# buwantaiji/FermiFlow

Hardware: AMD Instinct MI355X
Metric: walker-steps/sec (full VMC iteration: 100 MCMC steps + generate + E_loc + grad + Adam) (higher is better)
Workload: dtype f64

## Files before the change

### fermiflow_amd/csrc/ff_cnf_fwd.hip

```cpp
#include <atomic>
#include "ff_common.h"
#include "ff_ode.h"
#include "ff_slater.h"
#include "ff_eloc_ws.h"
#define FF_RADIAL_BUILD_KERNELS
#include "ff_radial.h"

#ifdef FF_STAMPS
#define FF_STAMP(i) do { unsigned long long t_ = __builtin_amdgcn_s_memtime(); stamp_acc[i] += t_ - stamp_prev; stamp_prev = t_; } while (0)
#else
#define FF_STAMP(i) do { } while (0)
#endif

#ifndef FF_TAB_MODE
#define FF_TAB_MODE(MODE) true
#endif

#include "ff_fwd_args.h"

#ifndef FF_FORM_EARLY
#define FF_FORM_EARLY 1
#endif
#ifndef FF_SWEEP_CH
#define FF_SWEEP_CH 2
#endif
#ifndef FF_FWD_WAVES_PER_SIMD
#define FF_FWD_WAVES_PER_SIMD 1
#endif
#ifndef FF_FLOW_WAVES
#define FF_FLOW_WAVES 3
#endif
#ifndef FF_FWD_STATIC
#define FF_FWD_STATIC(N, D, MODE, TAB) ((MODE) == 0 && (TAB) && (N) * (D) <= 12)
#endif
template <int N, int D, int MODE_, bool TAB>
__global__ void __launch_bounds__(FF_WAVE, ((MODE_ == 0 || MODE_ == FF_MODE_FRAMES) && TAB && N * D <= 12) ? FF_FLOW_WAVES : FF_FWD_WAVES_PER_SIMD)
ff_ode_fwd_kernel(ff_fwd_args A) {
  constexpr bool FRAMES = MODE_ == FF_MODE_FRAMES;
  constexpr int MODE = FRAMES ? 0 : MODE_;
  if constexpr (MODE == 0) FF_SETPRIO();
  using Gm = ff_geom<N, D>;
  constexpr int M = Gm::M, G = Gm::G, P = Gm::P, R = Gm::RA;
  constexpr int NH = MODE == 0 ? 1 : (MODE == 1 ? 2 : 4);
  constexpr int NV = MODE == 0 ? 1 : (MODE == 1 ? 2 : M + 5);
  constexpr int IDL = MODE == 1 ? 1 : M + 3;

  __shared__ ff_wtab s_w[TAB ? 1 : 2][TAB ? 1 : FF_HPAD];
  __shared__ double s_e2[TAB ? 1 : 64];
  __shared__ double s_z[G][M], s_kb[G][M], s_err[G][M];
  constexpr bool JET = (MODE == 2);
  __shared__ __attribute__((aligned(16))) double s_rr[JET ? 1 : G][JET ? 1 : R][2];
  __shared__ __attribute__((aligned(16))) double s_hd[JET ? 1 : G][JET ? 1 : R][NH];
  constexpr int RECW = (D + 7 + 1) & ~1;
  constexpr int RECS0 = R * RECW, RECS = RECS0 + ((RECS0 % 4 == 2) ? 0 : ((RECS0 % 4 == 0) ? 2 : 1));
  static_assert(!JET || ((2 * RECS) % 32) % 8 == 4, "record stride");
  __shared__ __attribute__((aligned(16))) double s_rec[JET ? G * RECS : 1];
  constexpr int QTW = ((3 * N > M) ? 3 * N + 1 : M + 1) | 1;
  constexpr int TROW = N * 3 * D + 1;
  static_assert(N * TROW <= M * QTW, "T must fit the transposition buffer");
  __shared__ __attribute__((aligned(16))) double s_qt[JET ? G * M * QTW : 1];
  __shared__ int s_pa[R], s_pb[R], s_any;
  __shared__ double s_rmin[G][R];
  static_assert(MODE != 2 || M <= 12, "the column-sweep local-energy kernel serves at most 12 coordinates");
  constexpr bool LDS_STATE = (MODE == 2);
  __shared__ double s_yv[LDS_STATE ? NV : 1][FF_WAVE], s_cv[LDS_STATE ? NV : 1][FF_WAVE];

  const int lane = threadIdx.x;
  const int g = lane / M, i = lane % M;
  const bool ingrp = g < G;
  const int gg = ingrp ? g : 0;
  const int ai = i / D, ci = i % D;
  const double* __restrict__ rtab = A.net.radial_table;
  if constexpr (TAB) {
    if (rtab[3] != 0.0) {
      if (lane == 0 && blockIdx.x == 0) *A.evt = A.evt_id;
      return;
    }
  } else {
    if (A.evt && *A.evt != A.evt_id) return;
    ff_fill_exp2_table(s_e2, lane);
    ff_load_weights(s_w, A.net, lane);
  }
  bool off_table = false;
  if (lane == 0) {
    int p = 0;
    for (int a = 0; a < N; a++)
      for (int b = a + 1; b < N; b++) { s_pa[p] = a; s_pb[p] = b; p++; }
    for (int a = 0; a < N; a++) { if (P + a < R) { s_pa[P + a] = a; s_pb[P + a] = -1; } }
  }
  FF_WG1_SYNC();
  const int He = A.net.He, Hm = A.net.Hm;
  const bool has_mu = Hm > 0;
  const int nrad = has_mu ? (P + N) : P;
  const double tab_inv_h = TAB ? rtab[0] : 0.0, tab_h = TAB ? rtab[1] : 0.0;
  auto heads = [&](int t, double r, double* hd) {
    if constexpr (TAB) {
      if (!ff_heads_table<NH>(rtab, tab_inv_h, tab_h, t, r, hd)) {
        off_table = true;
#pragma unroll
        for (int m = 0; m < NH; m++) hd[m] = 0.0;
      }
    } else {
      ff_heads<NH, FF_TAB_MODE(MODE)>(s_w[t], s_e2, t ? Hm : He, r, hd);
    }
  };
  const double rtol = A.rtol, atol = A.atol;
  constexpr double NT = MODE == 0 ? M : (MODE == 1 ? M + 1 : M * (M + 4) + 1);
  const int64_t ngroups = (A.B + G - 1) / G;
  __shared__ int s_st[4];
  if (lane < 4) s_st[lane] = 0;
  constexpr int NQ = (G * R + FF_WAVE - 1) / FF_WAVE;
  int rq_id[NQ];
#pragma unroll
  for (int qk = 0; qk < NQ; qk++) {
    const int q = lane + qk * FF_WAVE;
    const bool act = q < G * nrad;
// ... 74 lines not shown
        case 2: g0 = h * FF_A20; g1 = h * FF_A21; break;
        case 3: g0 = h * FF_A30; g1 = h * FF_A31; g2 = h * FF_A32; break;
        case 4: gy = 0.0; g0 = 1.0; break;
        case 5: gy = 0.0; g1 = 1.0; break;
        case 6: gy = 0.0; g2 = 1.0; break;
        default: break;
      }
      auto form = [&](double* dst, const int v0, const int v1, const int stride) {
#pragma unroll
        for (int v = v0; v < v1; v += stride) dst[v] = fma(g2, c2[v], fma(g1, c1[v], fma(g0, c0[v], gy * y[v])));
      };
      FF_STAMP(0);
      FF_WG1_SYNC();
      {
        double pub[NV];
        form(pub, 0, MODE == 2 ? M + 2 : 1, MODE == 2 ? M + 1 : 1);
        if (ingrp) {
          s_z[g][i] = pub[0];
          if constexpr (MODE == 2) s_kb[g][i] = pub[M + 1];
        }
      }
      FF_WG1_SYNC();
      FF_STAMP(1);
      double rq_rho[NQ][D], rq_dk[JET ? NQ : 1][D], rq_r[NQ], rq_ri[NQ], rq_T[NQ][TAB ? NH + 5 : 1], rq_dr[NQ];
      bool rq_ok[NQ];
#pragma unroll
      for (int qk = 0; qk < NQ; qk++) {
        const int id = rq_id[qk];
        const bool act = id >= 0;
        const int qg = act ? (id & 15) : 0, a = act ? ((id >> 4) & 15) : 0, bq = act ? ((id >> 8) & 15) : 15;
        const bool pair = bq != 15;
        const int bb = pair ? bq : a;
        double r2 = 0.0;
#pragma unroll
        for (int c = 0; c < D; c++) {
          rq_rho[qk][c] = s_z[qg][a * D + c] - (pair ? s_z[qg][bb * D + c] : 0.0);
          if constexpr (JET) rq_dk[qk][c] = s_kb[qg][a * D + c] - (pair ? s_kb[qg][bb * D + c] : 0.0);
          r2 = fma(rq_rho[qk][c], rq_rho[qk][c], r2);
        }
        ff_sqrt_rcp(r2, rq_r[qk], rq_ri[qk]);
        if (act) rmin_q[qk] = fmin(rmin_q[qk], rq_r[qk]);
        rq_dr[qk] = 0.0;
        rq_ok[qk] = true;
        if constexpr (TAB) {
          rq_ok[qk] = ff_table_fetch<NH>(rtab, tab_inv_h, tab_h, pair ? 0 : 1, rq_r[qk], rq_T[qk], rq_dr[qk]);
          if (act && !rq_ok[qk]) off_table = true;
        }
      }
      double in[NV], out[NV];
      if constexpr (MODE == 2 && FF_FORM_EARLY) form(in, 0, NV, 1);
#pragma unroll
      for (int qk = 0; qk < NQ; qk++) {
        const int id = rq_id[qk];
        if (id < 0) break;
        const int qg = id & 15, a = (id >> 4) & 15, bq = (id >> 8) & 15, p = id >> 12;
        const bool pair = bq != 15;
        const int bb = pair ? bq : a;
        const double* rho = rq_rho[qk];
        const double r = rq_r[qk], ri = rq_ri[qk];
        double hd[NH];
        if constexpr (TAB) {
          if (rq_ok[qk]) ff_table_eval<NH>(rq_T[qk], rq_dr[qk], hd);
          else {
#pragma unroll
            for (int m = 0; m < NH; m++) hd[m] = 0.0;
          }
        } else {
          heads(pair ? 0 : 1, r, hd);
        }
        if constexpr (!JET) {
          s_rr[qg][p][0] = r;
          s_rr[qg][p][1] = ri;
#pragma unroll
          for (int m = 0; m < NH; m++) s_hd[qg][p][m] = hd[m];
        } else {
          const double cf = pair ? 2.0 : 1.0;
          const double f0 = hd[0], f1 = hd[1], f2 = hd[NH > 2 ? 2 : 0], f3 = hd[NH > 3 ? 3 : 0];
          const double Ac = cf * fma(f2, r, (1.0 + D) * f1), Bc = cf * fma(f3, r, (2.0 + D) * f2);
          double* rec = &s_rec[qg * RECS + p * RECW];
#pragma unroll
          for (int c = 0; c < D; c++) rec[c] = rho[c];
          rec[D] = ri; rec[D + 1] = f0; rec[D + 2] = f1; rec[D + 3] = f2; rec[D + 4] = Ac; rec[D + 5] = Bc;
          rec[D + 6] = cf * fma(f1, r, D * f0);
          const double* dk = rq_dk[qk];
          double rdk = 0.0;
#pragma unroll
          for (int c = 0; c < D; c++) rdk = fma(rho[c], dk[c], rdk);
          const double F1k = f1 * (rdk * ri), gq = Ac * ri;
          double* Ta = &s_qt[qg * M * QTW + a * TROW + bb * 3 * D];
          double* Tb = &s_qt[qg * M * QTW + bb * TROW + a * 3 * D];
#pragma unroll
          for (int c = 0; c < D; c++) {
            const double pv = f0 * rho[c], pw = fma(F1k, rho[c], f0 * dk[c]), pg = gq * rho[c];
            Ta[c] = pv; Ta[D + c] = pw; Ta[2 * D + c] = pg;
            if (pair) { Tb[c] = -pv; Tb[D + c] = -pw; Tb[2 * D + c] = -pg; }
          }
        }
      }
      FF_WG1_SYNC();
      nev++;
      FF_STAMP(2);
      if constexpr (!(MODE == 2 && FF_FORM_EARLY)) form(in, 0, NV, 1);
      FF_STAMP(6);
      const double* sz = s_z[gg];
      double sumq = 0.0, ddiv = 0.0, qdiv = 0.0, divv = 0.0;
// ... 58 lines not shown
                if (pair) { du[bq * D + cc] -= g1; qv[bq * D + cc] -= g2; }
              }
              ddiv = fma(Ac, r1, ddiv);
              qdiv = fma(Bc, r1s, fma(Ac, r2q, qdiv));
              divv += hq[D + 6];
            }
          }
          FF_SCHED_FENCE();
        }
        FF_STAMP(7);
#pragma unroll
        for (int k = 0; k < M; k++) out[1 + k] = du[k];
        if (ingrp) {
#pragma unroll
          for (int k = 0; k < M; k++) s_qt[(g * M + i) * QTW + k] = qv[k];
        }
        FF_WG1_SYNC();
#pragma unroll
        for (int j = 0; j < M; j++) sumq += s_qt[(gg * M + j) * QTW + i];
        FF_STAMP(3);
      } else {
        if constexpr (MODE == 1) {
          for (int p = 0; p < nrad; p++) {
            const double c = p < P ? 2.0 : 1.0;
            divv = fma(c, fma(s_hd[gg][p][NH > 1 ? 1 : 0], s_rr[gg][p][0], D * s_hd[gg][p][0]), divv);
          }
        }
        const double zc = sz[ai * D + ci];
#pragma unroll
        for (int bq = 0; bq < N; bq++) {
          const bool self = (bq == ai);
          const int lo = bq < ai ? bq : ai, hi = bq < ai ? ai : bq;
          const int p = self ? 0 : ff_pair_index(N, lo, hi);
          vi = fma(self ? 0.0 : s_hd[gg][p][0], zc - sz[bq * D + ci], vi);
        }
        if (has_mu) vi = fma(s_hd[gg][P + ai][0], zc, vi);
      }
      out[0] = vi;
      if constexpr (MODE == 1) out[1] = -divv;
      if constexpr (MODE == 2) {
        out[M + 1] = sumq + dvk;
        out[M + 2] = -ddiv;
        out[M + 3] = -divv;
        out[M + 4] = -fma(gdi, in[M + 1], qdiv);
      }
      FF_STAMP(4);
#if defined(FF_STAMPS) && defined(FF_STAMPS_TRACE)
      const int s_prev = sv;
#endif
      if (sv == -2) {
#pragma unroll
        for (int v = 0; v < NV; v++) c0[v] = out[v];
        double p0 = 0.0, p1 = 0.0;
#pragma unroll
        for (int v = 0; v < NV; v++) {
          const double isc = wgt(v) * ff_rcp(fma(fabs(y[v]), rtol, atol));
          p0 = fma(y[v] * isc, y[v] * isc, p0);
          p1 = fma(c0[v] * isc, c0[v] * isc, p1);
        }
        const double d0 = sqrt(group_sum(p0) * (1.0 / NT));
        d1v = sqrt(group_sum(p1) * (1.0 / NT));
        h0v = S.h0(d0, d1v);
        s = -1;
        if (!ff_wave_or(&s_any, lane, (!S.done && !warm) ? 1 : 0)) {
          S.habs = fmin(hwarm, S.interval);
          S.plan();
          s = 1;
// ... 1165 lines not shown
```

### fermiflow_amd/csrc/ff_common.h

```cpp
#pragma once
#include <stdint.h>
#include <math.h>
#include "../../include/fermiflow.h"

#define FF_WAVE 64
#define FF_MAX_ORB 36
#define FF_MAX_NS 12
#define FF_HMAX 256
#define FF_HPAD (FF_HMAX + 8)

#ifdef FF_HOSTSIM
#include "../../tests/hostsim/hip_shim.h"
#else
#include <hip/hip_runtime.h>
#define FF_LAUNCH(kernel, grid, block, stream, ...) \
  hipLaunchKernelGGL(kernel, dim3(grid), dim3(block), 0, (hipStream_t)(stream), __VA_ARGS__)
#define FF_LAUNCH_LDS(kernel, grid, block, lds_bytes, stream, ...) \
  hipLaunchKernelGGL(kernel, dim3(grid), dim3(block), (lds_bytes), (hipStream_t)(stream), __VA_ARGS__)
#define FF_DYN_LDS(name) extern __shared__ double name[]
#endif

#ifndef FF_WAVE_SYNC
#define FF_WAVE_SYNC() do { __builtin_amdgcn_fence(__ATOMIC_RELEASE, "workgroup"); __builtin_amdgcn_wave_barrier(); \
                            __builtin_amdgcn_fence(__ATOMIC_ACQUIRE, "workgroup"); } while (0)
// ... 287 lines not shown
  p = fma(p, z, 1.0 / 3.0);
  p = fma(p, z, 1.0);
  const double ef = (double)e;
  return fma(ef, 6.93147180369123816490e-01, fma(2.0 * s, p, ef * 1.90821492927058770002e-10));
}

FF_D void ff_sincospi(double t, double* sn, double* cs) {
  const double q = rint(t * 2.0);
  const double r = fma(q, -0.5, t) * 3.14159265358979323846;
  const double r2 = r * r;
  double ps = -1.0 / 1307674368000.0;
  ps = fma(ps, r2, 1.0 / 6227020800.0);
  ps = fma(ps, r2, -1.0 / 39916800.0);
  ps = fma(ps, r2, 1.0 / 362880.0);
  ps = fma(ps, r2, -1.0 / 5040.0);
  ps = fma(ps, r2, 1.0 / 120.0);
  ps = fma(ps, r2, -1.0 / 6.0);
  ps = fma(ps * r2, r, r);
  double pc = 1.0 / 20922789888000.0;
  pc = fma(pc, r2, -1.0 / 87178291200.0);
  pc = fma(pc, r2, 1.0 / 479001600.0);
  pc = fma(pc, r2, -1.0 / 3628800.0);
  pc = fma(pc, r2, 1.0 / 40320.0);
  pc = fma(pc, r2, -1.0 / 720.0);
  pc = fma(pc, r2, 1.0 / 24.0);
  pc = fma(pc, r2, -0.5);
  pc = fma(pc, r2, 1.0);
  const int k = ((int)q) & 3;
  const double s0 = (k & 1) ? pc : ps, c0 = (k & 1) ? ps : pc;
  *sn = (k & 2) ? -s0 : s0;
  *cs = ((k + 1) & 2) ? -c0 : c0;
}

FF_HD int ff_pair_index(int n, int i, int j) { return i * (2 * n - i - 1) / 2 + (j - i - 1); }
```

### fermiflow_amd/csrc/ff_mcmc.h

```cpp
#pragma once
#include "ff_common.h"
#include "ff_slater.h"
#include "ff_rng.h"

FF_D double ff_mul_rn(double a, double b) { double r = a * b; FF_OPAQUE(r); return r; }
FF_D double ff_add_rn(double a, double b) { double r = a + b; FF_OPAQUE(r); return r; }
template <int N>
FF_D void ff_propose(const double* x, double tau, const double* z, double* nx) {
#pragma unroll
  for (int i = 0; i < N; i++) nx[i] = ff_add_rn(x[i], ff_mul_rn(tau, z[i]));
}

FF_D double ff_accept_prob(double dlp) { return !(dlp == dlp) ? dlp : (dlp < -708.0 ? 0.0 : ff_exp(fmin(dlp, 708.0))); }

FF_D bool ff_ratio_accept(double u, double dRt, double P2, double Pn2) {
  const double lhs = u * ff_exp(fmin(fmax(-dRt, -700.0), 708.0)) * P2;
  return (dRt >= -708.0) & (lhs < Pn2);
}

struct ff_mc_head { int64_t b; int sub; bool live; uint64_t wid; int md; };

template <int LPW, int N0, int N1>
FF_D ff_mc_head ff_mc_preamble(int64_t B, const int* __restrict__ tab_up, const int* __restrict__ tab_dn, const int* __restrict__ wstate,
                               int64_t woff, int* o0, int* o1) {
  static_assert(LPW == 1 || LPW == 2, "one or two lanes per walker");
  __shared__ int s_md;
  const int64_t gid = (int64_t)blockIdx.x * blockDim.x + threadIdx.x;
  ff_mc_head w;
  w.b = LPW == 2 ? gid >> 1 : gid;
  w.sub = LPW == 2 ? (int)(gid & 1) : 0;
  if (threadIdx.x == 0) s_md = 0;
  __syncthreads();
  w.live = w.b < B;
  if (!w.live) w.b = B - 1;
  const int st = wstate ? wstate[w.b] : 0;
  const int* __restrict__ tab = w.sub ? tab_dn : tab_up;
  int md = 0;
#pragma unroll
  for (int j = 0; j < N0; j++) ff_orb_decode(tab[st * N0 + j], o0[j], o0[N0 + j]);
#pragma unroll
  for (int j = 0; j < N1; j++) ff_orb_decode(tab_dn[st * N1 + j], o1[j], o1[N1 + j]);
#pragma unroll
  for (int j = 0; j < 2 * N0; j++) md = o0[j] > md ? o0[j] : md;
#pragma unroll
  for (int j = 0; j < 2 * N1; j++) md = o1[j] > md ? o1[j] : md;
  atomicMax(&s_md, md);
  __syncthreads();
  w.md = FF_UNIFORM(s_md);
  w.wid = (uint64_t)(woff + w.b);
  return w;
}

template <bool NOISE, class Layout>
FF_D void ff_mc_init(const Layout& L, const double* __restrict__ g0, double* x) {
  if (NOISE || g0 != nullptr) {
    L.load(g0 + L.w.b * Layout::M, x);
  } else {
    double u0;
    L.draw(0u, x, u0);
  }
}

template <class Layout>
FF_D void ff_mc_store(const Layout& L, const double* x, double logp, int nacc, double* __restrict__ x_out, double* __restrict__ logp_out,
                      int* __restrict__ acc_count) {
  if (!L.w.live) return;
  L.store(x_out + L.w.b * Layout::M, x);
  if (L.w.sub == 0) {
    if (logp_out) logp_out[L.w.b] = logp;
    if (acc_count) acc_count[L.w.b] = nacc;
  }
}

template <bool NOISE, class Layout>
FF_D void ff_mc_logp_chain(const Layout& L, int64_t B, int steps, double tau, const double* __restrict__ g0, const double* __restrict__ g,
                           const double* __restrict__ u, double* __restrict__ x_out, double* __restrict__ logp_out,
                           uint8_t* __restrict__ accept, int* __restrict__ acc_count) {
  constexpr int MS = Layout::MS, M = Layout::M;
  const int64_t b = L.w.b;
  double x[MS], nx[MS];
  ff_mc_init<NOISE>(L, g0, x);
// ... 62 lines not shown
template <int NU, int ND>
struct ff_mc_one_lane {
  static_assert(NU > 0 && ND >= 0, "compile-time spin sizes");
  static constexpr int n = NU + ND, M = 2 * n, MS = M;
  ff_mc_head w;
  uint64_t seed;
  int ou[2 * NU], od[2 * (ND > 0 ? ND : 1)];
  FF_D void load(const double* __restrict__ row, double* dst) const {
#pragma unroll
    for (int i = 0; i < M; i++) dst[i] = row[i];
  }
  FF_D void store(double* __restrict__ row, const double* x) const {
#pragma unroll
    for (int i = 0; i < M; i++) row[i] = x[i];
  }
  FF_D void draw(uint32_t step, double* z, double& u) const {
#pragma unroll
    for (int q = 0; q < (M + 3) / 4; q++) {
      double z4[4];
      ff_normal_quad(seed, w.wid, step, (uint32_t)q, z4);
#pragma unroll
      for (int k = 0; k < 4; k++) if (4 * q + k < M) z[4 * q + k] = z4[k];
    }
    u = ff_uniform(seed, w.wid, step, (uint32_t)n);
  }
  FF_D double logprob(const double* x) const {
    double s = 0.0;
    s += ff_slater_logabsdet_reg<NU>(ou, ou + NU, x, w.md);
    if constexpr (ND > 0) s += ff_slater_logabsdet_reg<ND>(od, od + ND, x + 2 * NU, w.md);
    return 2.0 * s;
  }
};

template <int NS>
struct ff_mc_spin_lanes {
  static constexpr int MS = 2 * NS, M = 2 * MS, n = 2 * NS;
  static constexpr bool ODD = (NS & 1) != 0;
  static constexpr int MID = (NS - 1) / 2;
  static constexpr int NB = ODD ? (NS + 1) / 2 : NS / 2 + 1;
  ff_mc_head w;
  uint64_t seed;
  int oo[2 * NS];
  FF_D void load(const double* __restrict__ row, double* dst) const {
#pragma unroll
    for (int i = 0; i < MS; i++) dst[i] = row[w.sub * MS + i];
  }
  FF_D void store(double* __restrict__ row, const double* x) const {
#pragma unroll
    for (int i = 0; i < MS; i++) row[w.sub * MS + i] = x[i];
  }
  FF_D double logprob(const double* x) const {
    const double L = ff_slater_logabsdet_reg<NS>(oo, oo + NS, x, w.md);
    return 2.0 * (L + ff_swap1(L));
  }
  FF_D double r2sum(const double* x) const {
    double R = 0.0;
#pragma unroll
    for (int i = 0; i < MS; i++) R = fma(x[i], x[i], R);
    return R;
  }
  FF_D double polydet2(const double* x) const {
    const double P = ff_slater_polydet_reg<NS>(oo, oo + NS, x, w.md), PP = P * ff_swap1(P);
    return PP * PP;
  }
  FF_D void draw(uint32_t step, double* z, double& u) const {
    const int sp = w.sub;
    auto swap32 = [](uint32_t v) -> uint32_t { return (uint32_t)__builtin_amdgcn_mov_dpp((int)v, 0xB1, 0xF, 0xF, true); };
    ff_u4 R[NB];
#pragma unroll
    for (int k = 0; k < NB; k++) {
      uint32_t slot;
      if constexpr (ODD) slot = sp ? (uint32_t)(k < NB - 1 ? MID + 1 + k : n) : (uint32_t)k;
      else slot = (k < NB - 1) ? (uint32_t)(sp * (NS / 2) + k) : (uint32_t)n;
      R[k] = ff_philox(seed, w.wid, step, slot);
    }
    auto word = [&](int pair, int c) -> uint32_t {
      const ff_u4& r = R[pair >> 1];
      return (pair & 1) ? (c ? r.w : r.z) : (c ? r.y : r.x);
    };
    uint32_t uh, ul;
    if constexpr (ODD) {
      const ff_u4& last = R[NB - 1];
      const uint32_t r0 = swap32(sp ? last.x : last.z), r1 = swap32(sp ? last.y : last.w);
#pragma unroll
      for (int j = 0; j < NS; j++) {
        const uint32_t a0 = word(j, 0), a1 = word(j, 1);
        const uint32_t b0 = j == 0 ? r0 : word(j > 0 ? j - 1 : 0, 0), b1 = j == 0 ? r1 : word(j > 0 ? j - 1 : 0, 1);
        ff_normal_pair32(sp ? b0 : a0, sp ? b1 : a1, z[2 * j], z[2 * j + 1]);
      }
      uh = sp ? last.x : r0; ul = sp ? last.y : r1;
    } else {
#pragma unroll
      for (int j = 0; j < NS; j++) ff_normal_pair32(word(j, 0), word(j, 1), z[2 * j], z[2 * j + 1]);
      uh = R[NB - 1].x; ul = R[NB - 1].y;
    }
    u = ff_uniform_words(uh, ul);
  }
};

template <int NS>
struct ff_mc_pair_lanes {
  static constexpr int M = 2 * NS, NQT = (NS + 1) / 2, NQL = (NQT + 1) / 2, NPL = 2 * NQL, MS = 2 * NPL;
  ff_mc_head w;
  uint64_t seed;
  int oo[2 * NS];
  FF_D int pid(int sl) const { return 4 * (sl >> 1) + 2 * w.sub + (sl & 1); }
  FF_D void load(const double* __restrict__ row, double* dst) const {
#pragma unroll
    for (int sl = 0; sl < NPL; sl++) {
      const int p = pid(sl) < NS ? pid(sl) : 0;
      dst[2 * sl] = row[2 * p]; dst[2 * sl + 1] = row[2 * p + 1];
    }
  }
  FF_D void store(double* __restrict__ row, const double* x) const {
#pragma unroll
    for (int sl = 0; sl < NPL; sl++) {
      if (pid(sl) < NS) { row[2 * pid(sl)] = x[2 * sl]; row[2 * pid(sl) + 1] = x[2 * sl + 1]; }
    }
  }
  FF_D void draw(uint32_t step, double* z, double& u) const {
#pragma unroll
    for (int k = 0; k < NQL; k++) ff_normal_quad(seed, w.wid, step, (uint32_t)(2 * k + w.sub), z + 4 * k);
    u = ff_uniform(seed, w.wid, step, (uint32_t)NS);
  }
  FF_D void gather(const double (&Dm)[NPL][NS], double (&Dfull)[NS][NS]) const {
#pragma unroll
    for (int i = 0; i < NS; i++) {
      const int q = i >> 1, owner = q & 1, sl = 2 * (q >> 1) + (i & 1);
#pragma unroll
      for (int j = 0; j < NS; j++) {
        const double mine = Dm[sl][j], other = ff_swap1(mine);
        Dfull[i][j] = (w.sub == owner) ? mine : other;
      }
    }
  }
  FF_D double logprob(const double* xs) const {
    double Dm[NPL][NS], Dfull[NS][NS];
#pragma unroll
    for (int sl = 0; sl < NPL; sl++) ff_slater_row_reg<NS>(oo, oo + NS, xs[2 * sl], xs[2 * sl + 1], w.md, Dm[sl]);
    gather(Dm, Dfull);
    return 2.0 * (0.0 + ff_lu_logabsdet_reg<NS>(Dfull));
  }
  FF_D double polydet2(const double* xs) const {
    double Dm[NPL][NS], Dfull[NS][NS];
#pragma unroll
    for (int sl = 0; sl < NPL; sl++) ff_poly_row_reg<NS>(oo, oo + NS, xs[2 * sl], xs[2 * sl + 1], w.md, Dm[sl]);
    gather(Dm, Dfull);
    const double P = ff_det_reg<NS>(Dfull);
    return P * P;
  }
  FF_D double r2sum(const double* xs) const {
    double r = 0.0;
#pragma unroll
    for (int sl = 0; sl < NPL; sl++) { const double t = fma(xs[2 * sl], xs[2 * sl], xs[2 * sl + 1] * xs[2 * sl + 1]); r += (pid(sl) < NS) ? t : 0.0; }
    return r;
  }
};

#ifdef FF_MCMC_BUILD_KERNELS
template <int NU, int ND, bool NOISE>
__global__ void __launch_bounds__(128)
ff_mcmc_kernel(int64_t B, int nup_rt, int ndn_rt, const int* __restrict__ tab_up, const int* __restrict__ tab_dn,
               const int* __restrict__ wstate, int steps, double tau,
               const double* __restrict__ g0, const double* __restrict__ g, const double* __restrict__ u,
               uint64_t seed, int64_t woff,
               double* __restrict__ x_out, double* __restrict__ logp_out, uint8_t* __restrict__ accept,
               int* __restrict__ acc_count) {
  ff_mc_one_lane<NU, ND> L;
  L.w = ff_mc_preamble<1, NU, ND>(B, tab_up, tab_dn, wstate, woff, L.ou, L.od);
  L.seed = seed;
  ff_mc_logp_chain<NOISE>(L, B, steps, tau, g0, g, u, x_out, logp_out, accept, acc_count);
}

template <int NS, bool NOISE>
__global__ void __launch_bounds__(128)
ff_mcmc_spin_kernel(int64_t B, const int* __restrict__ tab_up, const int* __restrict__ tab_dn, const int* __restrict__ wstate,
                    int steps, double tau, const double* __restrict__ g0, const double* __restrict__ g,
                    const double* __restrict__ u, uint64_t seed, int64_t woff, double* __restrict__ x_out,
                    double* __restrict__ logp_out, uint8_t* __restrict__ accept, int* __restrict__ acc_count) {
  static_assert(NOISE, "the Philox-fed chain of this layout is ff_mcmc_spin_philox_kernel<NS>");
  ff_mc_spin_lanes<NS> L;
  L.w = ff_mc_preamble<2, NS, 0>(B, tab_up, tab_dn, wstate, woff, L.oo, nullptr);
  L.seed = seed;
  ff_mc_logp_chain<true>(L, B, steps, tau, g0, g, u, x_out, logp_out, accept, acc_count);
}

template <int NS>
__global__ void __launch_bounds__(128)
ff_mcmc_spin_philox_kernel(int64_t B, const int* __restrict__ tab_up, const int* __restrict__ tab_dn, const int* __restrict__ wstate,
                           int steps, double tau, const double* __restrict__ g0, uint64_t seed, int64_t woff,
                           double* __restrict__ x_out, double* __restrict__ logp_out, int* __restrict__ acc_count) {
  ff_mc_spin_lanes<NS> L;
  L.w = ff_mc_preamble<2, NS, 0>(B, tab_up, tab_dn, wstate, woff, L.oo, nullptr);
  L.seed = seed;
  ff_mc_ratio_chain(L, steps, tau, g0, x_out, logp_out, acc_count);
}

template <int NS, bool NOISE>
__global__ void __launch_bounds__(128)
ff_mcmc_pair_kernel(int64_t B, const int* __restrict__ tab_up, const int* __restrict__ wstate, int steps, double tau,
                    const double* __restrict__ g0, const double* __restrict__ g, const double* __restrict__ u, uint64_t seed,
                    int64_t woff, double* __restrict__ x_out, double* __restrict__ logp_out, uint8_t* __restrict__ accept,
                    int* __restrict__ acc_count) {
  ff_mc_pair_lanes<NS> L;
  L.w = ff_mc_preamble<2, NS, 0>(B, tab_up, tab_up, wstate, woff, L.oo, nullptr);
  L.seed = seed;
  if constexpr (NOISE) ff_mc_logp_chain<true>(L, B, steps, tau, g0, g, u, x_out, logp_out, accept, acc_count);
  else ff_mc_ratio_chain(L, steps, tau, g0, x_out, logp_out, acc_count);
}

__global__ void __launch_bounds__(128)
ff_rng_fill_kernel(int64_t B, int n, int steps, uint64_t seed, int64_t woff, double* __restrict__ g0,
                   double* __restrict__ g, double* __restrict__ u) {
  int64_t b = (int64_t)blockIdx.x * blockDim.x + threadIdx.x;
  if (b >= B) return;
  const int M = 2 * n;
  const uint64_t wid = (uint64_t)(woff + b);
  for (int q = 0; 2 * q < n; q++) {
    double z4[4];
    ff_normal_quad(seed, wid, 0u, (uint32_t)q, z4);
    for (int k = 0; k < 4; k++) if (4 * q + k < M) g0[b * M + 4 * q + k] = z4[k];
  }
  for (int s = 0; s < steps; s++) {
    double* gs = g + ((int64_t)s * B + b) * M;
    for (int q = 0; 2 * q < n; q++) {
      double z4[4];
      ff_normal_quad(seed, wid, (uint32_t)(s + 1), (uint32_t)q, z4);
      for (int k = 0; k < 4; k++) if (4 * q + k < M) gs[4 * q + k] = z4[k];
    }
    u[(int64_t)s * B + b] = ff_uniform(seed, wid, (uint32_t)(s + 1), (uint32_t)n);
  }
}
#endif
```

### fermiflow_amd/csrc/ff_radial.h

```cpp
#pragma once
#include "ff_common.h"

#define FF_TAB_RMAX 32.0
#ifndef FF_TAB_ROW
#define FF_TAB_ROW 10
#endif
#define FF_TAB_MAXLOG 9
#define FF_TAB_NMAX (32 * (1 << FF_TAB_MAXLOG) + 1)
#define FF_TAB_HDR 16
#define FF_TAB_EVT0 8
#define FF_TAB_NEVT 8
#define FF_TAB_DOUBLES (FF_TAB_HDR + 2 * FF_TAB_NMAX * FF_TAB_ROW)

#define FF_SIGPOLY_INIT { \
    {0, 1, 0, 0, 0, 0, 0, 0, 0, 0, 0, 0, 0, 0}, \
    {0, 1, -1, 0, 0, 0, 0, 0, 0, 0, 0, 0, 0, 0}, \
    {0, 1, -3, 2, 0, 0, 0, 0, 0, 0, 0, 0, 0, 0}, \
    {0, 1, -7, 12, -6, 0, 0, 0, 0, 0, 0, 0, 0, 0}, \
    {0, 1, -15, 50, -60, 24, 0, 0, 0, 0, 0, 0, 0, 0}, \
    {0, 1, -31, 180, -390, 360, -120, 0, 0, 0, 0, 0, 0, 0}, \
    {0, 1, -63, 602, -2100, 3360, -2520, 720, 0, 0, 0, 0, 0, 0}, \
    {0, 1, -127, 1932, -10206, 25200, -31920, 20160, -5040, 0, 0, 0, 0, 0}, \
    {0, 1, -255, 6050, -46620, 166824, -317520, 332640, -181440, 40320, 0, 0, 0, 0}, \
    {0, 1, -511, 18660, -204630, 1020600, -2739240, 4233600, -3780000, 1814400, -362880, 0, 0, 0}, \
// ... 96 lines not shown
    for (int n = 0; n < 9; n++) {
      acc[n] += ff_swap1(acc[n]);
      acc[n] += ff_swap2(acc[n]);
    }
    if (live && part == 0) {
      double* row = tab + FF_TAB_HDR + ((size_t)t * FF_TAB_NMAX + j) * FF_TAB_ROW;
#pragma unroll
      for (int n = 0; n < 9 && n < FF_TAB_ROW; n++) row[n] = acc[n];
#pragma unroll
      for (int n = 9; n < FF_TAB_ROW; n++) row[n] = 0.0;
    }
  }
}

#endif

template <int NH>
FF_D bool ff_table_fetch(const double* __restrict__ tab, double inv_h, double h, int t, double r, double* T, double& dr) {
  if (!(r < FF_TAB_RMAX)) return false;
  const double jf = rint(r * inv_h);
  dr = fma(-jf, h, r);
#ifdef FF_DIAG_TAB_ROW0
  const double* __restrict__ row = tab + FF_TAB_HDR + ((size_t)t * FF_TAB_NMAX + 100) * FF_TAB_ROW;
#else
  const double* __restrict__ row = tab + FF_TAB_HDR + ((size_t)t * FF_TAB_NMAX + (int)jf) * FF_TAB_ROW;
#endif
  constexpr int NT = NH + 5 < FF_TAB_ROW ? NH + 5 : FF_TAB_ROW;
#pragma unroll
  for (int e = 0; e < NT; e++) T[e] = row[e];
  return true;
}

template <int NH>
FF_D void ff_table_eval(const double* T, double dr, double* hd) {
  constexpr int NT = NH + 5 < FF_TAB_ROW ? NH + 5 : FF_TAB_ROW;
  const double dk[5] = {dr, dr * 0.5, dr * (1.0 / 3.0), dr * 0.25, dr * 0.2};
#pragma unroll
  for (int m = 0; m < NH; m++) {
    const int top = m + 5 < NT ? m + 5 : NT - 1;
    double v = T[top];
#pragma unroll
    for (int k = 4; k >= 0; k--)
      if (m + k < top) v = fma(v, dk[k], T[m + k]);
    hd[m] = v;
  }
}

template <int NH>
FF_D bool ff_heads_table(const double* __restrict__ tab, double inv_h, double h, int t, double r, double* hd) {
  double T[NH + 5], dr;
  if (!ff_table_fetch<NH>(tab, inv_h, h, t, r, T, dr)) return false;
  ff_table_eval<NH>(T, dr, hd);
  return true;
}
```

### fermiflow_amd/csrc/ff_rng.h

```cpp
#pragma once
#include "ff_common.h"

struct ff_u4 { uint32_t x, y, z, w; };

FF_D ff_u4 ff_philox(uint64_t key, uint64_t c01, uint32_t c2, uint32_t c3) {
  uint32_t k0 = (uint32_t)key, k1 = (uint32_t)(key >> 32);
  uint32_t c0 = (uint32_t)c01, c1 = (uint32_t)(c01 >> 32);
#pragma unroll
  for (int r = 0; r < 10; r++) {
    uint64_t p0 = (uint64_t)0xD2511F53u * c0, p1 = (uint64_t)0xCD9E8D57u * c2;
    uint32_t n0 = (uint32_t)(p1 >> 32) ^ c1 ^ k0, n1 = (uint32_t)p1;
    uint32_t n2 = (uint32_t)(p0 >> 32) ^ c3 ^ k1, n3 = (uint32_t)p0;
    c0 = n0; c1 = n1; c2 = n2; c3 = n3;
    k0 += 0x9E3779B9u; k1 += 0xBB67AE85u;
  }
  ff_u4 o = {c0, c1, c2, c3};
  return o;
}

FF_D uint64_t ff_bits53(uint32_t hi, uint32_t lo) { return (((uint64_t)hi << 32) | lo) >> 11; }

FF_D void ff_normal_pair32(uint32_t a, uint32_t b, double& z0, double& z1) {
  const float u1 = fmaf((float)a, 2.3283064365386963e-10f, 1.1641532182693481e-10f);
  const float rad = __builtin_amdgcn_sqrtf(-1.3862943611198906f * __builtin_amdgcn_logf(u1));
  const float phi = (float)(b >> 2) * 2.3283064365386963e-10f;
  const float c = rad * __builtin_amdgcn_cosf(phi), s = rad * __builtin_amdgcn_sinf(phi);
  z0 = (double)__uint_as_float(__float_as_uint(c) ^ (b << 31));
  z1 = (double)__uint_as_float(__float_as_uint(s) ^ ((b << 30) & 0x80000000u));
}

FF_D void ff_normal_quad(uint64_t key, uint64_t walker, uint32_t step, uint32_t quad, double* z) {
  ff_u4 r = ff_philox(key, walker, step, quad);
  ff_normal_pair32(r.x, r.y, z[0], z[1]);
  ff_normal_pair32(r.z, r.w, z[2], z[3]);
}

FF_D double ff_uniform_words(uint32_t hi, uint32_t lo) { return (double)ff_bits53(hi, lo) * 1.1102230246251565e-16; }
FF_D double ff_uniform(uint64_t key, uint64_t walker, uint32_t step, uint32_t slot) {
  ff_u4 r = ff_philox(key, walker, step, slot);
  return ff_uniform_words(r.x, r.y);
}
```

### fermiflow_amd/csrc/ff_slater.h

```cpp
#pragma once
#include "ff_common.h"

__constant__ double FF_HERM_A[8][8] = {
    {1, 0, 0, 0, 0, 0, 0, 0},
    {0, 1, 0, 0, 0, 0, 0, 0},
    {-1, 0, 2, 0, 0, 0, 0, 0},
    {0, -3, 0, 2, 0, 0, 0, 0},
    {1.5, 0, -6, 0, 2, 0, 0, 0},
    {0, 7.5, 0, -10, 0, 2, 0, 0},
    {-1.25, 0, 7.5, 0, -5, 0, 2.0 / 3.0, 0},
    {0, -17.5, 0, 35, 0, -14, 0, 4.0 / 3.0}};
__constant__ double FF_HERM_NORM[8] = {
    1.0, 1.4142135623730951 , 0.70710678118654746 , 0.57735026918962584 ,
    0.40824829046386307 , 0.25819888974716110 , 0.44721359549995793 ,
    0.11952286093343936 };
#define FF_PI_SQRT_INV 0.56418958354775628

FF_D void ff_orb_decode(int k, int& nx, int& ny) {
  int shell = 0;
  while ((shell + 1) * (shell + 2) / 2 <= k) shell++;
  nx = k - shell * (shell + 1) / 2;
  ny = shell - nx;
}

// ... 182 lines not shown
    return fma(D[0][0], m0, fma(-D[0][1], m1, D[0][2] * m2));
  } else return ff_lu_absdet_reg<NS>(D);
}

template <int NS>
FF_D void ff_herm_rec_n(const int* n, double x, int md, double* res) {
  double hm = 1.0, h = FF_REC_A[0] * x;
#pragma unroll
  for (int j = 0; j < NS; j++) res[j] = (n[j] == 0) ? 1.0 : h;
  for (int m = 1; m < md; m++) {
    const double hn = fma(FF_REC_A[m] * x, h, -FF_REC_B[m] * hm);
    hm = h;
    h = hn;
#pragma unroll
    for (int j = 0; j < NS; j++) res[j] = (n[j] == m + 1) ? h : res[j];
  }
}
template <int NS>
FF_D void ff_poly_row_reg(const int* nx, const int* ny, double x, double y, int md, double* row) {
  double hy[NS];
  ff_herm_rec_n<NS>(nx, x, md, row);
  ff_herm_rec_n<NS>(ny, y, md, hy);
#pragma unroll
  for (int j = 0; j < NS; j++) row[j] *= hy[j];
}
template <int NS>
FF_D double ff_slater_polydet_reg(const int* nx, const int* ny, const double* x, int md) {
  double D[NS][NS];
#pragma unroll
  for (int i = 0; i < NS; i++) ff_poly_row_reg<NS>(nx, ny, x[2 * i], x[2 * i + 1], md, D[i]);
  return ff_det_reg<NS>(D);
}

template <int NS>
FF_D void ff_slater_row_reg(const int* nx, const int* ny, double x, double y, int md, double* row) {
  double gs = ff_gauss_of_r2(fma(x, x, y * y));
#pragma unroll
  for (int j = 0; j < NS; j++) row[j] = gs * ff_herm_rec(nx[j], x, md) * ff_herm_rec(ny[j], y, md);
}

template <int NS>
FF_D double ff_slater_logabsdet_reg(const int* nx, const int* ny, const double* x, int md) {
  double D[NS][NS];
#pragma unroll
  for (int i = 0; i < NS; i++) ff_slater_row_reg<NS>(nx, ny, x[2 * i], x[2 * i + 1], md, D[i]);
  return ff_lu_logabsdet_reg<NS>(D);
}

FF_D double ff_slater_general(int ns, const int* __restrict__ orb, const double* x,
                              double* T , double* S ) {
  double A[FF_MAX_NS * FF_MAX_NS], Inv[FF_MAX_NS * FF_MAX_NS];
  for (int i = 0; i < ns; i++) {
    double gs = ff_gauss2d(x[2 * i], x[2 * i + 1]);
    for (int j = 0; j < ns; j++) {
      double v;
      ff_orbital<false>(orb[j], x[2 * i], x[2 * i + 1], gs, v, nullptr, nullptr);
      A[i * ns + j] = v;
      Inv[i * ns + j] = (i == j) ? 1.0 : 0.0;
    }
  }
  double acc = 0.0;
  for (int c = 0; c < ns; c++) {
    int p = c;
    double best = fabs(A[c * ns + c]);
    for (int r = c + 1; r < ns; r++) {
      double a = fabs(A[r * ns + c]);
// ... 138 lines not shown
```

### fermiflow_amd/csrc/ff_walkers.hip

```cpp
#include <stdlib.h>
#include "ff_common.h"
#include "ff_slater.h"
#include "ff_rng.h"

#define FF_MAX_N 24

#define FF_MCMC_BUILD_KERNELS
#include "ff_mcmc.h"

__global__ void __launch_bounds__(128)
ff_slater_fwd_kernel(int64_t B, int n, const int* __restrict__ tab, const int* __restrict__ wstate,
                     const double* __restrict__ x, double* __restrict__ lad) {
  int64_t b = (int64_t)blockIdx.x * blockDim.x + threadIdx.x;
  if (b >= B) return;
  double xl[2 * FF_MAX_NS];
  for (int i = 0; i < 2 * n; i++) xl[i] = x[b * 2 * n + i];
  lad[b] = ff_slater_general(n, tab + (wstate ? wstate[b] : 0) * n, xl, nullptr, nullptr);
}

__global__ void __launch_bounds__(128)
ff_slater_bwd_kernel(int64_t B, int n, const int* __restrict__ tab, const int* __restrict__ wstate,
                     const double* __restrict__ x, const double* __restrict__ gout, double* __restrict__ gx) {
  int64_t b = (int64_t)blockIdx.x * blockDim.x + threadIdx.x;
  if (b >= B) return;
// ... 557 lines not shown
  const double d = buf[0] / n;
  const double E = c0 + d, Ess = buf[1] - buf[0] * d, F = sF / n;
  const double dF = sD / n;
  const double Fss = buf[1] + 2.0 * sCE + sCC - sD * dF;
  double sG = 0.0, sC = 0.0, sT = 0.0;
  for (int s = t; s < Ns; s += nt) {
    double se = 0.0, cnt = 0.0, sl = 0.0, sle = 0.0;
    for (int k = 0; k < FF_SS_K; k++) { const double* o = part + ((size_t)s * FF_SS_K + k) * 4; se += o[0]; cnt += o[1]; sl += o[2]; sle += o[3]; }
    const double lp = logits[s] - lz;
    const double cF = (se + cnt * lp / beta - cnt * F) / n;
    gphi[s] = cF;
    sG += lp * cF; sC += cF;
    sT += sle - (se / fmax(cnt, 1.0)) * sl;
  }
  sG = block_sum(sG); sC = block_sum(sC); sT = block_sum(sT);
  for (int s = t; s < Ns; s += nt) gphi[s] -= exp(logits[s] - lz) * sC;
  if (t == 0) {
    est[0] = E; est[1] = Ess < 0.0 ? 0.0 : Ess; est[2] = F; est[3] = Fss < 0.0 ? 0.0 : Fss; est[4] = -sS / n; est[5] = -sSa; est[6] = sG; est[7] = sT / n;
  }
}

#include "ff_observe.h"

#include "ff_host.h"

template <int NU, int ND>
static void launch_mcmc(bool noise, void* stream, int64_t B, int nup, int ndn, const int* tu, const int* td, const int* ws,
                        int steps, double tau, const double* g0, const double* g, const double* u, uint64_t seed, int64_t woff,
                        double* x_out, double* logp_out, uint8_t* accept, int* acc_count) {
  if constexpr (NU == ND && NU >= 1 && NU <= 6) {
    if (noise)
      FF_LAUNCH((ff_mcmc_spin_kernel<NU, true>), ff_grid(2 * B, 128), 128, stream, B, tu, td, ws, steps, tau, g0, g, u, seed, woff,
                x_out, logp_out, accept, acc_count);
    else
      FF_LAUNCH((ff_mcmc_spin_philox_kernel<NU>), ff_grid(2 * B, 128), 128, stream, B, tu, td, ws, steps, tau, g0, seed, woff,
                x_out, logp_out, acc_count);
  } else if constexpr (ND == 0 && NU >= 2 && NU <= 6) {
    if (noise)
      FF_LAUNCH((ff_mcmc_pair_kernel<NU, true>), ff_grid(2 * B, 128), 128, stream, B, tu, ws, steps, tau, g0, g, u, seed, woff, x_out,
                logp_out, accept, acc_count);
    else
      FF_LAUNCH((ff_mcmc_pair_kernel<NU, false>), ff_grid(2 * B, 128), 128, stream, B, tu, ws, steps, tau, g0, g, u, seed, woff, x_out,
                logp_out, accept, acc_count);
  } else {
    if (noise)
      FF_LAUNCH((ff_mcmc_kernel<NU, ND, true>), ff_grid(B, 128), 128, stream, B, nup, ndn, tu, td, ws, steps, tau, g0, g, u, seed, woff,
                x_out, logp_out, accept, acc_count);
    else
      FF_LAUNCH((ff_mcmc_kernel<NU, ND, false>), ff_grid(B, 128), 128, stream, B, nup, ndn, tu, td, ws, steps, tau, g0, g, u, seed, woff,
                x_out, logp_out, accept, acc_count);
  }
}

extern int ff_mcmc_rows_launch(void* stream, int d, bool noise, int64_t B, int nup, int ndn, const int* tu, const int* td, const int* ws,
                               int steps, double tau, const double* g0, const double* g, const double* u, uint64_t seed, int64_t woff,
                               double* x_out, double* logp_out, uint8_t* accept, int* acc_count);

static int mcmc_dispatch(bool noise, void* stream, int64_t B, int nup, int ndn, const int* tu, const int* td, const int* ws,
                         int steps, double tau, const double* g0, const double* g, const double* u, uint64_t seed, int64_t woff,
                         double* x_out, double* logp_out, uint8_t* accept, int* acc_count) {
  FF_CHECK(B >= 0 && nup >= 0 && ndn >= 0 && nup + ndn > 0 && steps >= 0, FF_EINVAL, "ff_mcmc: bad sizes");
  if (const int st = ff_check_det_size("ff_mcmc", nup, ndn)) return st;
  FF_CHECK(x_out && (nup == 0 || tu) && (ndn == 0 || td), FF_EINVAL, "ff_mcmc: null pointer");
  FF_CHECK(!noise || (g0 && (steps == 0 || (g && u))), FF_EINVAL, "ff_mcmc: null noise pointer");
  if (B == 0) return FF_OK;
#define FF_MC(NU_, ND_) if (nup == NU_ && ndn == ND_) { launch_mcmc<NU_, ND_>(noise, stream, B, nup, ndn, tu, td, ws, steps, tau, g0, g, u, seed, woff, x_out, logp_out, accept, acc_count); FF_LAUNCH_CHECK(); return FF_OK; }
  FF_MC(3, 3) FF_MC(3, 0) FF_MC(6, 0) FF_MC(6, 6) FF_MC(1, 0) FF_MC(2, 0) FF_MC(4, 0)
  FF_MC(1, 1) FF_MC(2, 2) FF_MC(4, 4) FF_MC(5, 5) FF_MC(5, 0) FF_MC(10, 0)
#undef FF_MC
  return ff_mcmc_rows_launch(stream, 2, noise, B, nup, ndn, tu, td, ws, steps, tau, g0, g, u, seed, woff, x_out, logp_out, accept, acc_count);
}

#define FF_ORD_BINS 32
#define FF_ORD_THREADS 256
#define FF_ORD_SEG 512
FF_D int ff_ord_row(int c) { return FF_ORD_BINS - 1 - (c < 0 ? 0 : (c > FF_ORD_BINS - 1 ? FF_ORD_BINS - 1 : c)); }
// ... 519 lines not shown
```

Measured before the change: 6.140 billion.

## Specialize MCMC for ground-state orbitals and streamline tabulated flow forward

```diff
diff --git a/fermiflow_amd/csrc/ff_cnf_fwd.hip b/fermiflow_amd/csrc/ff_cnf_fwd.hip
--- a/fermiflow_amd/csrc/ff_cnf_fwd.hip
+++ b/fermiflow_amd/csrc/ff_cnf_fwd.hip
@@ -49,7 +49,8 @@
   __shared__ double s_e2[TAB ? 1 : 64];
   __shared__ double s_z[G][M], s_kb[G][M], s_err[G][M];
   constexpr bool JET = (MODE == 2);
-  __shared__ __attribute__((aligned(16))) double s_rr[JET ? 1 : G][JET ? 1 : R][2];
+  constexpr bool LEAN = (MODE == 0 && TAB);
+  __shared__ __attribute__((aligned(16))) double s_rr[(JET || LEAN) ? 1 : G][(JET || LEAN) ? 1 : R][2];
   __shared__ __attribute__((aligned(16))) double s_hd[JET ? 1 : G][JET ? 1 : R][NH];
   constexpr int RECW = (D + 7 + 1) & ~1;
   constexpr int RECS0 = R * RECW, RECS = RECS0 + ((RECS0 % 4 == 2) ? 0 : ((RECS0 % 4 == 0) ? 2 : 1));
@@ -59,6 +60,7 @@
   constexpr int TROW = N * 3 * D + 1;
   static_assert(N * TROW <= M * QTW, "T must fit the transposition buffer");
   __shared__ __attribute__((aligned(16))) double s_qt[JET ? G * M * QTW : 1];
+  __shared__ double s_zero[LEAN ? (D > 2 ? D : 2) : 1];
   __shared__ int s_pa[R], s_pb[R], s_any;
   __shared__ double s_rmin[G][R];
   static_assert(MODE != 2 || M <= 12, "the column-sweep local-energy kernel serves at most 12 coordinates");
@@ -82,6 +84,7 @@
     ff_load_weights(s_w, A.net, lane);
   }
   bool off_table = false;
+  if constexpr (LEAN) { if (lane < (D > 2 ? D : 2)) s_zero[lane] = 0.0; }
   if (lane == 0) {
     int p = 0;
     for (int a = 0; a < N; a++)
@@ -222,9 +225,11 @@
         const bool pair = bq != 15;
         const int bb = pair ? bq : a;
         double r2 = 0.0;
+        const double* zpart = pair ? &s_z[qg][bb * D] : s_zero;
 #pragma unroll
         for (int c = 0; c < D; c++) {
-          rq_rho[qk][c] = s_z[qg][a * D + c] - (pair ? s_z[qg][bb * D + c] : 0.0);
+          if constexpr (LEAN) rq_rho[qk][c] = s_z[qg][a * D + c] - zpart[c];
+          else rq_rho[qk][c] = s_z[qg][a * D + c] - (pair ? s_z[qg][bb * D + c] : 0.0);
           if constexpr (JET) rq_dk[qk][c] = s_kb[qg][a * D + c] - (pair ? s_kb[qg][bb * D + c] : 0.0);
           r2 = fma(rq_rho[qk][c], rq_rho[qk][c], r2);
         }
@@ -233,8 +238,13 @@
         rq_dr[qk] = 0.0;
         rq_ok[qk] = true;
         if constexpr (TAB) {
-          rq_ok[qk] = ff_table_fetch<NH>(rtab, tab_inv_h, tab_h, pair ? 0 : 1, rq_r[qk], rq_T[qk], rq_dr[qk]);
-          if (act && !rq_ok[qk]) off_table = true;
+          if constexpr (LEAN) {
+            rq_ok[qk] = ff_table_fetch_always<NH>(rtab, tab_inv_h, tab_h, pair ? 0 : 1, rq_r[qk], rq_T[qk], rq_dr[qk]);
+            off_table |= act & !rq_ok[qk];
+          } else {
+            rq_ok[qk] = ff_table_fetch<NH>(rtab, tab_inv_h, tab_h, pair ? 0 : 1, rq_r[qk], rq_T[qk], rq_dr[qk]);
+            if (act && !rq_ok[qk]) off_table = true;
+          }
         }
       }
       double in[NV], out[NV];
@@ -249,7 +259,11 @@
         const double* rho = rq_rho[qk];
         const double r = rq_r[qk], ri = rq_ri[qk];
         double hd[NH];
-        if constexpr (TAB) {
+        if constexpr (LEAN) {
+          ff_table_eval<NH>(rq_T[qk], rq_dr[qk], hd);
+#pragma unroll
+          for (int m = 0; m < NH; m++) hd[m] = rq_ok[qk] ? hd[m] : 0.0;
+        } else if constexpr (TAB) {
           if (rq_ok[qk]) ff_table_eval<NH>(rq_T[qk], rq_dr[qk], hd);
           else {
 #pragma unroll
@@ -259,8 +273,10 @@
           heads(pair ? 0 : 1, r, hd);
         }
         if constexpr (!JET) {
-          s_rr[qg][p][0] = r;
-          s_rr[qg][p][1] = ri;
+          if constexpr (!LEAN) {
+            s_rr[qg][p][0] = r;
+            s_rr[qg][p][1] = ri;
+          }
 #pragma unroll
           for (int m = 0; m < NH; m++) s_hd[qg][p][m] = hd[m];
         } else {
@@ -385,7 +401,12 @@
           const bool self = (bq == ai);
           const int lo = bq < ai ? bq : ai, hi = bq < ai ? ai : bq;
           const int p = self ? 0 : ff_pair_index(N, lo, hi);
-          vi = fma(self ? 0.0 : s_hd[gg][p][0], zc - sz[bq * D + ci], vi);
+          if constexpr (LEAN) {
+            const double* hp = self ? s_zero : &s_hd[gg][p][0];
+            vi = fma(*hp, zc - sz[bq * D + ci], vi);
+          } else {
+            vi = fma(self ? 0.0 : s_hd[gg][p][0], zc - sz[bq * D + ci], vi);
+          }
         }
         if (has_mu) vi = fma(s_hd[gg][P + ai][0], zc, vi);
       }
diff --git a/fermiflow_amd/csrc/ff_common.h b/fermiflow_amd/csrc/ff_common.h
--- a/fermiflow_amd/csrc/ff_common.h
+++ b/fermiflow_amd/csrc/ff_common.h
@@ -343,4 +343,12 @@
   *cs = ((k + 1) & 2) ? -c0 : c0;
 }
 
+FF_D uint32_t ff_xor3(uint32_t a, uint32_t b, uint32_t c) {
+#if defined(__HIP_DEVICE_COMPILE__) && defined(__gfx950__)
+  return (uint32_t)__builtin_amdgcn_bitop3_b32(a, b, c, 0x96);
+#else
+  return a ^ b ^ c;
+#endif
+}
+
 FF_HD int ff_pair_index(int n, int i, int j) { return i * (2 * n - i - 1) / 2 + (j - i - 1); }
diff --git a/fermiflow_amd/csrc/ff_mcmc.h b/fermiflow_amd/csrc/ff_mcmc.h
--- a/fermiflow_amd/csrc/ff_mcmc.h
+++ b/fermiflow_amd/csrc/ff_mcmc.h
@@ -47,6 +47,29 @@
   atomicMax(&s_md, md);
   __syncthreads();
   w.md = FF_UNIFORM(s_md);
+  w.wid = (uint64_t)(woff + w.b);
+  return w;
+}
+
+template <int NS>
+FF_D bool ff_mc_is_ground(const int* __restrict__ tab_a, const int* __restrict__ tab_b, const int* __restrict__ wstate) {
+  int bad = wstate != nullptr ? 1 : 0;
+#pragma unroll
+  for (int j = 0; j < NS; j++) bad |= (tab_a[j] ^ j) | (tab_b[j] ^ j);
+  return FF_UNIFORM(bad) == 0;
+}
+template <int LPW, int NS>
+FF_D ff_mc_head ff_mc_preamble_ground(int64_t B, int64_t woff, int* o0) {
+  static_assert(LPW == 2, "the two-lanes-per-walker layouts");
+  const int64_t gid = (int64_t)blockIdx.x * blockDim.x + threadIdx.x;
+  ff_mc_head w;
+  w.b = gid >> 1;
+  w.sub = (int)(gid & 1);
+  w.live = w.b < B;
+  if (!w.live) w.b = B - 1;
+#pragma unroll
+  for (int j = 0; j < NS; j++) { o0[j] = ff_ground_nx(j); o0[NS + j] = ff_ground_ny(j); }
+  w.md = ff_ground_md(NS);
   w.wid = (uint64_t)(woff + w.b);
   return w;
 }
@@ -175,7 +198,7 @@
   }
 };
 
-template <int NS>
+template <int NS, bool GROUND = false>
 struct ff_mc_spin_lanes {
   static constexpr int MS = 2 * NS, M = 2 * MS, n = 2 * NS;
   static constexpr bool ODD = (NS & 1) != 0;
@@ -203,7 +226,10 @@
     return R;
   }
   FF_D double polydet2(const double* x) const {
-    const double P = ff_slater_polydet_reg<NS>(oo, oo + NS, x, w.md), PP = P * ff_swap1(P);
+    double P;
+    if constexpr (GROUND) P = ff_slater_polydet_ground<NS>(x);
+    else P = ff_slater_polydet_reg<NS>(oo, oo + NS, x, w.md);
+    const double PP = P * ff_swap1(P);
     return PP * PP;
   }
   FF_D void draw(uint32_t step, double* z, double& u) const {
@@ -241,7 +267,7 @@
   }
 };
 
-template <int NS>
+template <int NS, bool GROUND = false>
 struct ff_mc_pair_lanes {
   static constexpr int M = 2 * NS, NQT = (NS + 1) / 2, NQL = (NQT + 1) / 2, NPL = 2 * NQL, MS = 2 * NPL;
   ff_mc_head w;
@@ -287,7 +313,10 @@
   FF_D double polydet2(const double* xs) const {
     double Dm[NPL][NS], Dfull[NS][NS];
 #pragma unroll
-    for (int sl = 0; sl < NPL; sl++) ff_poly_row_reg<NS>(oo, oo + NS, xs[2 * sl], xs[2 * sl + 1], w.md, Dm[sl]);
+    for (int sl = 0; sl < NPL; sl++) {
+      if constexpr (GROUND) ff_poly_row_ground<NS>(xs[2 * sl], xs[2 * sl + 1], Dm[sl]);
+      else ff_poly_row_reg<NS>(oo, oo + NS, xs[2 * sl], xs[2 * sl + 1], w.md, Dm[sl]);
+    }
     gather(Dm, Dfull);
     const double P = ff_det_reg<NS>(Dfull);
     return P * P;
@@ -321,32 +350,39 @@
                     int steps, double tau, const double* __restrict__ g0, const double* __restrict__ g,
                     const double* __restrict__ u, uint64_t seed, int64_t woff, double* __restrict__ x_out,
                     double* __restrict__ logp_out, uint8_t* __restrict__ accept, int* __restrict__ acc_count) {
-  static_assert(NOISE, "the Philox-fed chain of this layout is ff_mcmc_spin_philox_kernel<NS>");
+  static_assert(NOISE, "the Philox-fed chain of this layout is ff_mcmc_spin_philox_kernel<NS, GROUND>");
   ff_mc_spin_lanes<NS> L;
   L.w = ff_mc_preamble<2, NS, 0>(B, tab_up, tab_dn, wstate, woff, L.oo, nullptr);
   L.seed = seed;
   ff_mc_logp_chain<true>(L, B, steps, tau, g0, g, u, x_out, logp_out, accept, acc_count);
 }
 
-template <int NS>
+template <int NS, bool GROUND>
 __global__ void __launch_bounds__(128)
 ff_mcmc_spin_philox_kernel(int64_t B, const int* __restrict__ tab_up, const int* __restrict__ tab_dn, const int* __restrict__ wstate,
                            int steps, double tau, const double* __restrict__ g0, uint64_t seed, int64_t woff,
                            double* __restrict__ x_out, double* __restrict__ logp_out, int* __restrict__ acc_count) {
-  ff_mc_spin_lanes<NS> L;
-  L.w = ff_mc_preamble<2, NS, 0>(B, tab_up, tab_dn, wstate, woff, L.oo, nullptr);
+  if (ff_mc_is_ground<NS>(tab_up, tab_dn, wstate) != GROUND) return;
+  ff_mc_spin_lanes<NS, GROUND> L;
+  if constexpr (GROUND) L.w = ff_mc_preamble_ground<2, NS>(B, woff, L.oo);
+  else L.w = ff_mc_preamble<2, NS, 0>(B, tab_up, tab_dn, wstate, woff, L.oo, nullptr);
   L.seed = seed;
   ff_mc_ratio_chain(L, steps, tau, g0, x_out, logp_out, acc_count);
 }
 
-template <int NS, bool NOISE>
+template <int NS, bool NOISE, bool GROUND = false>
 __global__ void __launch_bounds__(128)
 ff_mcmc_pair_kernel(int64_t B, const int* __restrict__ tab_up, const int* __restrict__ wstate, int steps, double tau,
                     const double* __restrict__ g0, const double* __restrict__ g, const double* __restrict__ u, uint64_t seed,
                     int64_t woff, double* __restrict__ x_out, double* __restrict__ logp_out, uint8_t* __restrict__ accept,
                     int* __restrict__ acc_count) {
-  ff_mc_pair_lanes<NS> L;
-  L.w = ff_mc_preamble<2, NS, 0>(B, tab_up, tab_up, wstate, woff, L.oo, nullptr);
+  static_assert(!(NOISE && GROUND), "the noise-fed chain is the reference's arithmetic for every launch");
+  if constexpr (!NOISE) {
+    if (ff_mc_is_ground<NS>(tab_up, tab_up, wstate) != GROUND) return;
+  }
+  ff_mc_pair_lanes<NS, GROUND> L;
+  if constexpr (GROUND) L.w = ff_mc_preamble_ground<2, NS>(B, woff, L.oo);
+  else L.w = ff_mc_preamble<2, NS, 0>(B, tab_up, tab_up, wstate, woff, L.oo, nullptr);
   L.seed = seed;
   if constexpr (NOISE) ff_mc_logp_chain<true>(L, B, steps, tau, g0, g, u, x_out, logp_out, accept, acc_count);
   else ff_mc_ratio_chain(L, steps, tau, g0, x_out, logp_out, acc_count);
diff --git a/fermiflow_amd/csrc/ff_radial.h b/fermiflow_amd/csrc/ff_radial.h
--- a/fermiflow_amd/csrc/ff_radial.h
+++ b/fermiflow_amd/csrc/ff_radial.h
@@ -152,6 +152,21 @@
 }
 
 template <int NH>
+FF_D bool ff_table_fetch_always(const double* __restrict__ tab, double inv_h, double h, int t, double r, double* T, double& dr) {
+  static_assert((uint64_t)(FF_TAB_HDR + 2 * (uint64_t)FF_TAB_NMAX * FF_TAB_ROW) * 8 < (1ull << 31), "32-bit row offsets");
+  const bool ok = r < FF_TAB_RMAX;
+  const double jf = rint(r * inv_h);
+  dr = fma(-jf, h, r);
+  const int j = (int)(ok ? jf : 0.0);
+  const uint32_t off = (uint32_t)(FF_TAB_HDR + (t * FF_TAB_NMAX + j) * FF_TAB_ROW) * 8u;
+  const double* __restrict__ row = (const double*)((const char*)tab + off);
+  constexpr int NT = NH + 5 < FF_TAB_ROW ? NH + 5 : FF_TAB_ROW;
+#pragma unroll
+  for (int e = 0; e < NT; e++) T[e] = row[e];
+  return ok;
+}
+
+template <int NH>
 FF_D void ff_table_eval(const double* T, double dr, double* hd) {
   constexpr int NT = NH + 5 < FF_TAB_ROW ? NH + 5 : FF_TAB_ROW;
   const double dk[5] = {dr, dr * 0.5, dr * (1.0 / 3.0), dr * 0.25, dr * 0.2};
diff --git a/fermiflow_amd/csrc/ff_rng.h b/fermiflow_amd/csrc/ff_rng.h
--- a/fermiflow_amd/csrc/ff_rng.h
+++ b/fermiflow_amd/csrc/ff_rng.h
@@ -9,8 +9,8 @@
 #pragma unroll
   for (int r = 0; r < 10; r++) {
     uint64_t p0 = (uint64_t)0xD2511F53u * c0, p1 = (uint64_t)0xCD9E8D57u * c2;
-    uint32_t n0 = (uint32_t)(p1 >> 32) ^ c1 ^ k0, n1 = (uint32_t)p1;
-    uint32_t n2 = (uint32_t)(p0 >> 32) ^ c3 ^ k1, n3 = (uint32_t)p0;
+    uint32_t n0 = ff_xor3((uint32_t)(p1 >> 32), c1, k0), n1 = (uint32_t)p1;
+    uint32_t n2 = ff_xor3((uint32_t)(p0 >> 32), c3, k1), n3 = (uint32_t)p0;
     c0 = n0; c1 = n1; c2 = n2; c3 = n3;
     k0 += 0x9E3779B9u; k1 += 0xBB67AE85u;
   }
diff --git a/fermiflow_amd/csrc/ff_slater.h b/fermiflow_amd/csrc/ff_slater.h
--- a/fermiflow_amd/csrc/ff_slater.h
+++ b/fermiflow_amd/csrc/ff_slater.h
@@ -238,6 +238,49 @@
   return ff_det_reg<NS>(D);
 }
 
+constexpr int ff_ground_shell(int k) { int s = 0; while ((s + 1) * (s + 2) / 2 <= k) s++; return s; }
+constexpr int ff_ground_nx(int k) { return k - ff_ground_shell(k) * (ff_ground_shell(k) + 1) / 2; }
+constexpr int ff_ground_ny(int k) { return ff_ground_shell(k) - ff_ground_nx(k); }
+constexpr int ff_ground_md(int ns) { return ns > 0 ? ff_ground_shell(ns - 1) : 0; }
+template <int MD>
+FF_D void ff_herm_lit(double x, double* h) {
+  constexpr double RA[7] = {1.4142135623730951, 1.0, 0.81649658092772603, 0.70710678118654752, 0.63245553203367588,
+                            0.57735026918962576, 0.53452248382484879};
+  constexpr double RB[7] = {0.0, 0.70710678118654752, 0.81649658092772603, 0.86602540378443865, 0.89442719099991588,
+                            0.91287092917527686, 0.92582009977255146};
+  static_assert(MD >= 0 && MD <= 7, "degrees of the 36 orbitals");
+  if constexpr (MD >= 1) h[1] = RA[0] * x;
+  if constexpr (MD >= 2) h[2] = fma(RA[1] * x, h[1], -RB[1]);
+#pragma unroll
+  for (int m = 2; m < MD; m++) h[m + 1] = fma(RA[m] * x, h[m], -RB[m] * h[m - 1]);
+}
+template <int J, int NS>
+FF_D void ff_poly_row_ground_from(const double* hx, const double* hy, double* row) {
+  if constexpr (J < NS) {
+    constexpr int nx = ff_ground_nx(J), ny = ff_ground_ny(J);
+    if constexpr (nx == 0 && ny == 0) row[J] = 1.0;
+    else if constexpr (nx == 0) row[J] = hy[ny];
+    else if constexpr (ny == 0) row[J] = hx[nx];
+    else row[J] = hx[nx] * hy[ny];
+    ff_poly_row_ground_from<J + 1, NS>(hx, hy, row);
+  }
+}
+template <int NS>
+FF_D void ff_poly_row_ground(double x, double y, double* row) {
+  constexpr int MD = ff_ground_md(NS);
+  double hx[MD + 1], hy[MD + 1];
+  ff_herm_lit<MD>(x, hx);
+  ff_herm_lit<MD>(y, hy);
+  ff_poly_row_ground_from<0, NS>(hx, hy, row);
+}
+template <int NS>
+FF_D double ff_slater_polydet_ground(const double* x) {
+  double D[NS][NS];
+#pragma unroll
+  for (int i = 0; i < NS; i++) ff_poly_row_ground<NS>(x[2 * i], x[2 * i + 1], D[i]);
+  return ff_det_reg<NS>(D);
+}
+
 template <int NS>
 FF_D void ff_slater_row_reg(const int* nx, const int* ny, double x, double y, int md, double* row) {
   double gs = ff_gauss_of_r2(fma(x, x, y * y));
diff --git a/fermiflow_amd/csrc/ff_walkers.hip b/fermiflow_amd/csrc/ff_walkers.hip
--- a/fermiflow_amd/csrc/ff_walkers.hip
+++ b/fermiflow_amd/csrc/ff_walkers.hip
@@ -613,16 +613,22 @@
     if (noise)
       FF_LAUNCH((ff_mcmc_spin_kernel<NU, true>), ff_grid(2 * B, 128), 128, stream, B, tu, td, ws, steps, tau, g0, g, u, seed, woff,
                 x_out, logp_out, accept, acc_count);
-    else
-      FF_LAUNCH((ff_mcmc_spin_philox_kernel<NU>), ff_grid(2 * B, 128), 128, stream, B, tu, td, ws, steps, tau, g0, seed, woff,
+    else {
+      FF_LAUNCH((ff_mcmc_spin_philox_kernel<NU, true>), ff_grid(2 * B, 128), 128, stream, B, tu, td, ws, steps, tau, g0, seed, woff,
                 x_out, logp_out, acc_count);
+      FF_LAUNCH((ff_mcmc_spin_philox_kernel<NU, false>), ff_grid(2 * B, 128), 128, stream, B, tu, td, ws, steps, tau, g0, seed, woff,
+                x_out, logp_out, acc_count);
+    }
   } else if constexpr (ND == 0 && NU >= 2 && NU <= 6) {
     if (noise)
       FF_LAUNCH((ff_mcmc_pair_kernel<NU, true>), ff_grid(2 * B, 128), 128, stream, B, tu, ws, steps, tau, g0, g, u, seed, woff, x_out,
                 logp_out, accept, acc_count);
-    else
-      FF_LAUNCH((ff_mcmc_pair_kernel<NU, false>), ff_grid(2 * B, 128), 128, stream, B, tu, ws, steps, tau, g0, g, u, seed, woff, x_out,
+    else {
+      FF_LAUNCH((ff_mcmc_pair_kernel<NU, false, true>), ff_grid(2 * B, 128), 128, stream, B, tu, ws, steps, tau, g0, g, u, seed, woff, x_out,
                 logp_out, accept, acc_count);
+      FF_LAUNCH((ff_mcmc_pair_kernel<NU, false, false>), ff_grid(2 * B, 128), 128, stream, B, tu, ws, steps, tau, g0, g, u, seed, woff, x_out,
+                logp_out, accept, acc_count);
+    }
   } else {
     if (noise)
       FF_LAUNCH((ff_mcmc_kernel<NU, ND, true>), ff_grid(B, 128), 128, stream, B, nup, ndn, tu, td, ws, steps, tau, g0, g, u, seed, woff,
```

Result: faster. 6.293 billion, median of 6 (+2.5%).
